# cure-lab/PnPInversion

Hardware: AMD Instinct MI355X
Metric: edited images/sec @ 512x512, 50 DDIM-inv + 50 denoise steps (higher is better)
Workload: dtype f16 (fp32 accumulate; latents / scheduler math fp32); 1 GPU; single 512x512 image per rank, SD-1.x (seeded synthetic weights), directinversion+p2p, faithful schedule: 650 UNet sample-forwards + 1 VAE encode + 5 VAE decodes per image, Refine+Reweight+LocalBlend controller; text K/V projected once per loop (not per forward); ddim_steps=50, schedule=lockstep

## Files before the change

include/pnpi.h:

```cpp
#ifndef PNPI_H
#define PNPI_H
#include <stddef.h>
#include <stdint.h>

#ifdef __cplusplus
extern "C" {
#endif

typedef struct pnpi_ctx pnpi_ctx;

typedef enum {
  PNPI_OK = 0,
  PNPI_EINVAL = -1,
  PNPI_ESHAPE = -2,
  PNPI_EHIP = -3,
  PNPI_ESTATE = -4,
  PNPI_ENOMEM = -5
} pnpi_status;

typedef struct {
  int in_channels, out_channels;
  int n_blocks;
  int block_out_channels[4];
  int block_has_attn[4];
// ... 188 lines not shown
int pnpi_op_adam_step(pnpi_ctx* ctx, float* p, float* m, float* v, const float* g, int n, int k, float lr, float inv_scale);
int pnpi_op_attention_bwd(pnpi_ctx* ctx, const void* q, int ldq, int q_off, const void* k, int ldk, int k_off, const void* v, int ldv,
                          int v_off, const void* d_o, int ldo, int heads, int Nq, int Nk, int Dp, int dh, float scale, int B, void* dq,
                          void* dk, void* dv, void* scratch, size_t scratch_bytes);
size_t pnpi_op_attention_bwd_scratch_bytes(int Nq, int Nk, int dh);

int pnpi_edit_loop_uncond_steps(pnpi_ctx* ctx, const float* x_T, int nimg, const float* context4, const pnpi_ctrl_desc* ctrl_host, int nsteps,
                                const int* timesteps_host, float guidance_scale, int prox, float quantile, const float* uncond_steps,
                                int uncond_first_only, float* latents_out);
int pnpi_edit_loop_uncond_steps_recon(pnpi_ctx* ctx, const float* x_T, int nimg, const float* context4, const pnpi_ctrl_desc* ctrl_host, int nsteps,
                                      const int* timesteps_host, float guidance_scale, int prox, float quantile, const float* uncond_steps,
                                      int uncond_first_only, const pnpi_recon_desc* recon, float* latents_out);
int pnpi_unet_context_grad(pnpi_ctx* ctx, const float* latents, int t, const float* context, const float* d_eps, float* eps_out,
                           float* d_context_out);
int pnpi_null_text_optimize(pnpi_ctx* ctx, const float* ddim_latents, const float* ctx_uncond, const float* ctx_cond, int nsteps,
                            const int* timesteps_host, float guidance_scale, int num_inner_steps, float epsilon, float* uncond_out,
                            int* iters_out_host, float* losses_out_host);
int pnpi_null_latent_calculate(pnpi_ctx* ctx, const float* ddim_latents, const float* context4, int nsteps, const int* timesteps_host,
                               float guidance_scale, int num_inner_steps, float epsilon, float* noise_loss_out, int* iters_out_host,
                               float* losses_out_host);
int pnpi_op_attention(pnpi_ctx* ctx, const void* q, int ldq, int q_off, const void* k, int ldk, int k_off, const void* vt,
                      int ldv, void* o, int ldo, int heads, int Nq, int Nk, int Dp, int dh, float scale,
                      const int* rows_dev , int nrows);
int pnpi_op_cross_edit(pnpi_ctx* ctx, const void* q, int ldq, int q_off, const void* k, int ldk, int k_off, const void* vt,
                       int ldv, void* o, int ldo, int heads, int Nq, int Nk, int Dp, int dh, float scale,
                       const int* pairs_dev, int npairs, const void* mmatT_f16, const float* c1, const float* c2,
                       const float* lb_alpha, float* lb_acc, int lb_slot0, int lb_nslots);
int pnpi_op_local_blend(pnpi_ctx* ctx, const float* lb_acc, int nslots, int map_hw, int lat_hw, int C, float th,
                        float* latents, int nimg);
int pnpi_op_local_blend_sub(pnpi_ctx* ctx, const float* lb_acc, int nslots, int map_hw, int lat_hw, int C, float th, float th_sub,
                            float* latents, int nimg);

#ifdef __cplusplus
}
#endif
#endif
```

pnpinversion_amd/_capi.py:

```python
import ctypes as C
import os

_HERE = os.path.dirname(os.path.abspath(__file__))
LIB_PATH = os.path.join(_HERE, "csrc", "libpnpi.so")

PNPI_OK, PNPI_EINVAL, PNPI_ESHAPE, PNPI_EHIP, PNPI_ESTATE, PNPI_ENOMEM = 0, -1, -2, -3, -4, -5


class ModelConfig(C.Structure):
    _fields_ = [
        ("in_channels", C.c_int), ("out_channels", C.c_int), ("n_blocks", C.c_int),
        ("block_out_channels", C.c_int * 4), ("block_has_attn", C.c_int * 4),
        ("layers_per_block", C.c_int), ("heads", C.c_int), ("cross_dim", C.c_int), ("ctx_len", C.c_int),
        ("sample_size", C.c_int), ("norm_groups", C.c_int), ("n_train_timesteps", C.c_int),
        ("vae_in_channels", C.c_int), ("vae_latent_channels", C.c_int), ("vae_n_blocks", C.c_int),
        ("vae_block_out_channels", C.c_int * 4), ("vae_layers_per_block", C.c_int), ("vae_norm_groups", C.c_int),
        ("clip_layers", C.c_int), ("clip_heads", C.c_int), ("clip_intermediate", C.c_int), ("clip_vocab", C.c_int),
    ]


class NamedTensor(C.Structure):
    _fields_ = [("name", C.c_char_p), ("data", C.c_void_p), ("dtype", C.c_int), ("ndim", C.c_int), ("shape", C.c_int64 * 4)]


# ... 83 lines not shown
    "pnpi_op_gemm_geglu": (_i, [_vp, _vp, _i, _vp, _i, _i, _i, _i, _vp, _vp, _i]),
    "pnpi_op_groupnorm": (_i, [_vp, _vp, _vp, _i, _i, _i, _i, _i, _f, _vp, _vp, _i, _vp]),
    "pnpi_op_layernorm": (_i, [_vp, _vp, _i, _i, _f, _vp, _vp, _vp]),
    "pnpi_op_geglu": (_i, [_vp, _vp, _i, _i, _vp]),
    "pnpi_op_softmax_rows": (_i, [_vp, _vp, _i, _i, _i]),
    "pnpi_op_layernorm_bwd": (_i, [_vp, _vp, _vp, _i, _i, _f, _vp, _vp]),
    "pnpi_op_groupnorm_bwd": (_i, [_vp, _vp, _vp, _i, _i, _i, _i, _i, _f, _vp, _vp, _i, _vp, _vp]),
    "pnpi_op_geglu_bwd": (_i, [_vp, _vp, _vp, _i, _i, _vp]),
    "pnpi_op_softmax_bwd_rows": (_i, [_vp, _vp, _vp, _i, _i, _i, _f, _vp]),
    "pnpi_op_accumulate": (_i, [_vp, _vp, _vp, C.c_size_t]),
    "pnpi_op_sumpool2x2": (_i, [_vp, _vp, _i, _i, _i, _i, _vp]),
    "pnpi_op_zero_stuff2": (_i, [_vp, _vp, _i, _i, _i, _i, _vp]),
    "pnpi_op_repack_dgrad": (_i, [_vp, _vp, _i, _i, _i, _vp]),
    "pnpi_op_null_text_loss": (_i, [_vp, _vp, _vp, _vp, _vp, _i, _f, _f, _f, _f, _vp, _vp]),
    "pnpi_op_adam_step": (_i, [_vp, _vp, _vp, _vp, _vp, _i, _i, _f, _f]),
    "pnpi_op_attention_bwd": (_i, [_vp, _vp, _i, _i, _vp, _i, _i, _vp, _i, _i, _vp, _i, _i, _i, _i, _i, _i, _f, _i, _vp, _vp, _vp, _vp, C.c_size_t]),
    "pnpi_op_attention_bwd_scratch_bytes": (C.c_size_t, [_i, _i, _i]),
    "pnpi_edit_loop_uncond_steps": (_i, [_vp, _vp, _i, _vp, _vp, _i, C.POINTER(C.c_int), _f, _i, _f, _vp, _i, _vp]),
    "pnpi_edit_loop_uncond_steps_recon": (_i, [_vp, _vp, _i, _vp, _vp, _i, C.POINTER(C.c_int), _f, _i, _f, _vp, _i, C.POINTER(ReconDesc), _vp]),
    "pnpi_unet_context_grad": (_i, [_vp, _vp, _i, _vp, _vp, _vp, _vp]),
    "pnpi_null_text_optimize": (_i, [_vp, _vp, _vp, _vp, _i, C.POINTER(C.c_int), _f, _i, _f, _vp, C.POINTER(C.c_int), C.POINTER(C.c_float)]),
    "pnpi_null_latent_calculate": (_i, [_vp, _vp, _vp, _i, C.POINTER(C.c_int), _f, _i, _f, _vp, C.POINTER(C.c_int), C.POINTER(C.c_float)]),
    "pnpi_op_attention": (_i, [_vp, _vp, _i, _i, _vp, _i, _i, _vp, _i, _vp, _i, _i, _i, _i, _i, _i, _f, _vp, _i]),
    "pnpi_op_cross_edit": (_i, [_vp, _vp, _i, _i, _vp, _i, _i, _vp, _i, _vp, _i, _i, _i, _i, _i, _i, _f, _vp, _i, _vp, _vp,
                                _vp, _vp, _vp, _i, _i]),
    "pnpi_op_local_blend": (_i, [_vp, _vp, _i, _i, _i, _i, _f, _vp, _i]),
    "pnpi_op_local_blend_sub": (_i, [_vp, _vp, _i, _i, _i, _i, _f, _f, _vp, _i]),
    "pnpi_ef_step_scalars": (_i, [_fp, _i, _f, _i, _i, _f, _fp]),
    "pnpi_ef_sample_xts": (_i, [_vp, _vp, _i, _vp, _sz, _i, _ip, _vp]),
    "pnpi_ef_noise_map": (_i, [_vp, _vp, _i, _f, _vp, _vp, _vp, _i, _sz, _i, _i, _f]),
    "pnpi_ef_reverse_step": (_i, [_vp, _vp, _vp, _vp, _i, _i, _sz, _fp, _i, _i, _f, _vp]),
    "pnpi_ef_invert": (_i, [_vp, _vp, _i, _vp, _vp, _vp, _f, _fp, _i, _ip, _vp, _vp]),
    "pnpi_ef_edit": (_i, [_vp, _vp, _vp, _i, _i, _vp, _fp, C.POINTER(CtrlDesc), _fp, _i, _i, _ip, _vp]),
}

_lib = None


class PnpiError(RuntimeError):
    def __init__(self, status, message):
        super().__init__("libpnpi status %d: %s" % (status, message))
        self.status = status


def load_library(path=None):
    global _lib
# ... 28 lines not shown
```

pnpinversion_amd/csrc/api.hip:

```cpp
#include <math.h>
#include <stdio.h>
#include <stdlib.h>
#include <string.h>

#include <algorithm>
#include <functional>
#include <memory>
#include <string>

#include "model.h"

static int g_text_kv = 1;
static int g_temb_cache = 1;

static int fail(pnpi_ctx* c, int status, const char* what) {
  c->err = what;
  return status;
}
static int fail_launch(pnpi_ctx* c, int code, const char* what) {
  char buf[640];
  if (code > 0) {
    snprintf(buf, sizeof(buf), "HIP error %d (%s) in %s", code, hipGetErrorString((hipError_t)code), what);
    c->err = buf;
    return PNPI_EHIP;
// ... 1055 lines not shown
                       int ups, int Ho, int Wo, const void* w, const float* bias, const void* res, int N, void* out, int force_cfg,
                       int force_split, float* stats_out, int* tile_rows_out) {
  if (!c || !stats_out || !tile_rows_out) return PNPI_EINVAL;
  GemmP p; gemm_defaults(p);
  p.x1 = (const half_t*)x1; p.x2 = (const half_t*)x2; p.C1 = C1; p.C2 = C2; p.ldx1 = C1; p.ldx2 = C2;
  p.B = B; p.H = H; p.W = W; p.Ho = Ho; p.Wo = Wo; p.ksize = ksize; p.stride = stride; p.pad = pad; p.ups = ups;
  p.K = ksize * ksize * (C1 + C2); p.w = (const half_t*)w; p.ldw = p.K; p.M = B * Ho * Wo; p.N = N;
  p.bias = bias; p.res = (const half_t*)res; p.ldres = N; p.out = (half_t*)out; p.ldo = N; p.stats = stats_out;
  CK(launch_igemm(p, c->splitk_ws, c->splitk_bytes, c->st, force_cfg, force_split, nullptr, tile_rows_out));
  return 0;
}
int pnpi_tile_table_lookup(int M, int N, int K, int ksize, int* cfg, int* split, int* entry_m) {
  return igemm_table_lookup(M, N, K, ksize, cfg, split, entry_m);
}
int pnpi_set_tuning(const char* key, int value) {
  if (!key) return PNPI_EINVAL;
  if (!strcmp(key, "text_kv")) { g_text_kv = value; return 0; }
  if (!strcmp(key, "temb_cache")) { g_temb_cache = value; return 0; }
  if (!strcmp(key, "gn_inline_rows")) { norm_set_tuning_gn_inline_rows(value); return 0; }
  if (!strcmp(key, "attn_vt_perm")) { g_vt_perm = value; return 0; }
  if (!strcmp(key, "attn_aug")) { g_attn_aug = value; return 0; }
  if (!strcmp(key, "attn_pipe")) return attn_set_tuning_pipe(value) == 0 ? 0 : PNPI_EINVAL;
  if (!strcmp(key, "gn_slab")) { g_gn_slab = value; return 0; }
  if (!strcmp(key, "op_attention_aug")) { g_op_attention_aug = value; return 0; }
  if (!strcmp(key, "op_attention_vt_perm")) { g_op_attention_vt_perm = value; return 0; }
  if (!strcmp(key, "attn_bwd_flash")) { g_attn_bwd_flash = value; return 0; }
  return igemm_set_tuning(key, value) == 0 ? 0 : PNPI_EINVAL;
}
int pnpi_op_gemm(pnpi_ctx* c, const void* a, int lda, const void* w, int ldw, int M, int N, int K, float alpha, const float* bias,
                 const void* res, void* out, int ldo, int vt_col0, void* outT, int vt_ld, int vt_f32, int rpb, int force_cfg,
                 int force_split) {
  GemmP p; gemm_defaults(p);
  p.x1 = (const half_t*)a; p.C1 = K; p.ldx1 = lda; p.B = 1; p.H = 1; p.W = M; p.Ho = 1; p.Wo = M; p.ksize = 1;
  p.w = (const half_t*)w; p.ldw = ldw; p.M = M; p.N = N; p.K = K; p.alpha = alpha; p.bias = bias; p.res = (const half_t*)res;
  p.ldres = N; p.out = (half_t*)out; p.ldo = ldo;
  if (outT) { p.outT = outT; p.vt_col0 = vt_col0; p.vt_ld = vt_ld; p.vt_f32 = vt_f32; p.rows_per_batch = rpb; }
  CK(launch_igemm(p, c->splitk_ws, c->splitk_bytes, c->st, force_cfg, force_split));
  return 0;
}
int pnpi_op_gemm_geglu(pnpi_ctx* c, const void* a, int lda, const void* w, int ldw, int M, int N, int K, const float* bias, void* out,
                       int ldo) {
  GemmP p; gemm_defaults(p);
  p.x1 = (const half_t*)a; p.C1 = K; p.ldx1 = lda; p.B = 1; p.H = 1; p.W = M; p.Ho = 1; p.Wo = M; p.ksize = 1;
  p.w = (const half_t*)w; p.ldw = ldw; p.M = M; p.N = N; p.K = K; p.bias = bias; p.out = (half_t*)out; p.ldo = ldo; p.geglu = 1;
  CK(launch_igemm(p, c->splitk_ws, c->splitk_bytes, c->st));
  return 0;
// ... 256 lines not shown
int pnpi_op_repack_dgrad(pnpi_ctx* c, const void* w, int N, int taps, int Cin, void* wd) {
  CK(launch_repack_dgrad((const half_t*)w, N, N, taps, Cin, (half_t*)wd, c->st));
  return 0;
}
int pnpi_op_null_text_loss(pnpi_ctx* c, const float* eps_u, const float* eps_c, const float* x, const float* target, int n, float w, float c_x,
                           float c_e, float grad_scale, void* d_eps_u, float* loss) {
  CK(launch_null_text_loss(eps_u, eps_c, x, target, n, w, c_x, c_e, grad_scale, (float*)d_eps_u, loss, c->st));
  return 0;
}
int pnpi_op_adam_step(pnpi_ctx* c, float* p, float* m, float* v, const float* g, int n, int k, float lr, float inv_scale) {
  CK(launch_adam_step(p, m, v, g, n, k, lr, inv_scale, c->st));
  return 0;
}
int pnpi_op_attention(pnpi_ctx* c, const void* q, int ldq, int q_off, const void* k, int ldk, int k_off, const void* vt, int ldv,
                      void* o, int ldo, int heads, int Nq, int Nk, int Dp, int dh, float scale, const int* rows_dev, int nrows) {
  AttnP a; a.q = (const half_t*)q; a.ldq = ldq; a.q_off = q_off; a.k = (const half_t*)k; a.ldk = ldk; a.k_off = k_off;
  a.vt = (const half_t*)vt; a.ldv = ldv; a.o = (half_t*)o; a.ldo = ldo; a.heads = heads; a.Nq = Nq; a.Nk = Nk; a.Dp = Dp; a.dh = dh;
  a.scale = scale; a.rows = rows_dev; a.nrows = nrows;
  a.vt_perm = (g_op_attention_vt_perm && attn_flash_uses_dma64(Dp, Nk, 0)) ? 1 : 0;
  a.aug = g_op_attention_aug;
  CK(launch_attn_flash(a, c->st));
  return 0;
}
int pnpi_op_cross_edit(pnpi_ctx* c, const void* q, int ldq, int q_off, const void* k, int ldk, int k_off, const void* vt, int ldv,
                       void* o, int ldo, int heads, int Nq, int Nk, int Dp, int dh, float scale, const int* pairs_dev, int npairs,
                       const void* mmatT, const float* c1, const float* c2, const float* lb_alpha, float* lb_acc, int lb_slot0,
                       int lb_nslots) {
  CrossEditP e; e.q = (const half_t*)q; e.ldq = ldq; e.q_off = q_off; e.k = (const half_t*)k; e.ldk = ldk; e.k_off = k_off;
  e.vt = (const half_t*)vt; e.ldv = ldv; e.o = (half_t*)o; e.ldo = ldo; e.heads = heads; e.Nq = Nq; e.Nk = Nk; e.Dp = Dp; e.dh = dh;
  e.scale = scale; e.pairs = pairs_dev; e.npairs = npairs; e.mmatT = (const half_t*)mmatT; e.c1 = c1; e.c2 = c2;
  e.lb_alpha = lb_alpha; e.lb_acc = lb_acc; e.lb_slot0 = lb_slot0; e.lb_nslots = lb_nslots; e.write_src = 1;
  CK(launch_attn_cross_edit(e, c->st));
  return 0;
}
int pnpi_op_local_blend(pnpi_ctx* c, const float* lb_acc, int nslots, int map_hw, int lat_hw, int C, float th, float* latents, int nimg) {
  CK(launch_local_blend(lb_acc, nslots, map_hw, lat_hw, C, th, latents, nimg, c->st));
  return 0;
}
int pnpi_op_local_blend_sub(pnpi_ctx* c, const float* lb_acc, int nslots, int map_hw, int lat_hw, int C, float th, float th_sub,
                            float* latents, int nimg) {
  CK(launch_local_blend(lb_acc, nslots, map_hw, lat_hw, C, th, latents, nimg, c->st, 4, th_sub));
  return 0;
}

}
```

pnpinversion_amd/csrc/api_ctrl.inc:

```
static void for_each_transformer(pnpi_ctx* c, const std::function<void(const TransformerW&, int)>& fn) {
  UNetW& u = c->unet;
  int idx = 0;
  for (auto& blk : u.down_attn) for (auto& t : blk) fn(t, idx++);
  fn(u.mid_attn, idx++);
  for (auto& blk : u.up_attn) for (auto& t : blk) fn(t, idx++);
}
static size_t text_kv_bytes(pnpi_ctx* c, int rows) {
  const int T = c->cfg.ctx_len, ldv = round_up_i(T, 8);
  size_t total = 0;
  for_each_transformer(c, [&](const TransformerW& t, int) {
    const size_t hd = (size_t)t.heads * t.Dp;
    total += align_up((size_t)rows * T * hd * sizeof(half_t), 256) + align_up((size_t)rows * hd * ldv * sizeof(half_t), 256);
  });
  return total + 4096;
}
static int text_kv_precompute(pnpi_ctx* c, const float* context, int rows) {
  const pnpi_model_config& g = c->cfg;
  TextKV& kv = c->tkv;
  kv.rows = 0; kv.use = false;
  if (rows <= 0 || rows > c->max_rows) return fail(c, PNPI_EINVAL, "text K/V precompute: rows out of range (max_unet_rows)");
  if (text_kv_bytes(c, rows) > kv.cap) return fail(c, PNPI_ENOMEM, "text K/V cache arena too small");
  const int T = g.ctx_len, X = g.cross_dim, ldv = round_up_i(T, 8);
  c->persist.reset(); c->temp.reset();
  half_t* ctx16 = palloc(c, (size_t)rows * T * X);
// ... 50 lines not shown
      if (step_list) step_on.assign(cds[i].masa_step_on_host, cds[i].masa_step_on_host + cds[i].masa_n_steps);
      if (cd.masa_any && (cd.masa_start_step != cds[i].masa_start_step || cd.masa_start_layer != cds[i].masa_start_layer ||
                          cd.masa_layer_mask != cds[i].masa_layer_mask || cd.masa_step_list != step_list || cd.masa_step_on != step_on))
        return fail(c, PNPI_EINVAL, "all MasaCtrl controllers of one batch must share their step / layer windows (or lists)");
      cd.masa_any = true; cd.masa_start_step = cds[i].masa_start_step; cd.masa_start_layer = cds[i].masa_start_layer;
      cd.masa_layer_mask = cds[i].masa_layer_mask; cd.masa_step_list = step_list; cd.masa_step_on = step_on;
      for (int half = 0; half < 2; ++half) {
        const int src = i * 4 + 2 * half, tgt = src + 1;
        masa[tgt * 4 + 2] = src; masa[tgt * 4 + 3] = src;
      }
    }
    if (cd.masa_any) {
      cd.rows_masa = (int*)c->ctrl_arena.alloc(masa.size() * sizeof(int));
      CKP(upload(c, cd.rows_masa, masa.data(), masa.size() * sizeof(int)));
    }
  }
  cd.any_edit = !edit_img.empty();
  cd.npairs = (int)edit_img.size();
  std::vector<bool> is_pair_row(rows, false);
  for (int i : edit_img) {
    int src = i * rpi + src_off, tgt = i * rpi + tgt_off;
    rep[tgt * 4 + 1] = src; rep[tgt * 4 + 2] = src;
    pairs.push_back(src); pairs.push_back(tgt);
    is_pair_row[tgt] = true;
    cd.pair_img.push_back(i);
  }
  for (int r = 0; r < rows; ++r) if (!is_pair_row[r]) { plain.push_back(r); plain.push_back(r); plain.push_back(r); plain.push_back(r); }
  cd.n_plain = (int)plain.size() / 4;
  cd.rows_id = (int*)c->ctrl_arena.alloc(id.size() * sizeof(int));
  cd.rows_rep = (int*)c->ctrl_arena.alloc(rep.size() * sizeof(int));
  CKP(upload(c, cd.rows_id, id.data(), id.size() * sizeof(int)));
  CKP(upload(c, cd.rows_rep, rep.data(), rep.size() * sizeof(int)));
  if (!plain.empty()) {
    cd.rows_plain = (int*)c->ctrl_arena.alloc(plain.size() * sizeof(int));
    CKP(upload(c, cd.rows_plain, plain.data(), plain.size() * sizeof(int)));
  }
  if (!cd.any_edit) return 0;
  cd.pairs = (int*)c->ctrl_arena.alloc(pairs.size() * sizeof(int));
  CKP(upload(c, cd.pairs, pairs.data(), pairs.size() * sizeof(int)));
  const pnpi_ctrl_desc& d0 = cds[edit_img[0]];
  cd.n_alpha_rows = d0.n_alpha_rows;
  cd.self_lo = d0.self_replace_lo; cd.self_hi = d0.self_replace_hi; cd.self_max_tokens = d0.self_replace_max_tokens;
  const int P = cd.npairs;
  std::vector<half_t> mm((size_t)P * 96 * 96, (half_t)0.f);
  int planes = 2;
  for (int pi = 0; pi < P; ++pi)
// ... 64 lines not shown
```

pnpinversion_amd/csrc/api_graph.inc:

```
static void prof_open(pnpi_ctx* c, ProfRec& r) {
  (void)hipEventCreate(&r.a); (void)hipEventCreate(&r.b);
  (void)hipEventRecord(r.a, c->st);
}
static void prof_close(pnpi_ctx* c, ProfRec& r, int cls, double flops, double bytes, int M = 0, int N = 0, int K = 0, int ks = 0) {
  (void)hipEventRecord(r.b, c->st);
  r.cls = cls; r.flops = flops; r.bytes = bytes; r.M = M; r.N = N; r.K = K; r.ksize = ks;
  c->prof.push_back(r);
}
static int g_gn_slab = 0;
static int flush_pending(pnpi_ctx* c) {
  if (!c->pend_on) return 0;
  c->pend_on = false;
  return launch_splitk_reduce(c->pend, c->st);
}
#define PROF(cls, flops, bytes, expr) PROFD(cls, flops, bytes, 0, 0, 0, expr)
#define PROFD(cls, flops, bytes, d0, d1, d2, expr)            \
  do {                                                        \
    if (c->pend_on) { int _f = flush_pending(c); if (_f) return fail_launch(c, _f, "deferred split-K combine"); } \
    if (c->prof_on && !c->dry) {                              \
      ProfRec _pr; prof_open(c, _pr);                         \
      int _r = (expr);                                        \
      prof_close(c, _pr, (cls), (flops), (bytes), (d0), (d1), (d2)); \
      if (_r) return fail_launch(c, _r, #expr);               \
    } else {                                                  \
// ... 15 lines not shown
  const NormW* nw = nullptr;
  int G = 0, HW = 0, silu = 0;
  float eps = 0.f;
  const half_t *q = nullptr, *k = nullptr, *v = nullptr;
  const float* lse = nullptr;
  int ldq = 0, q_off = 0, ldk = 0, k_off = 0, ldv = 0, v_off = 0, heads = 0, Nq = 0, Nk = 0, Dp = 0, dh = 0;
  float scale = 0.f;
};
struct Tape {
  std::vector<TapeOp> ops;
  bool rec = false;
  const half_t* no_grad_input = nullptr;
  const half_t* ctx16 = nullptr;
  Bump garena;
  std::unordered_map<const void*, half_t*> grads;
  std::unordered_map<const void*, half_t*> wd;
  float* d_ctx = nullptr;
  void* attn_scratch = nullptr; size_t attn_scratch_bytes = 0;
};
static int g_attn_aug = 1;
static int g_vt_perm = 1;
static int g_attn_bwd_flash = 1;
static int g_op_attention_aug = 0;
static int g_op_attention_vt_perm = 0;
static inline bool taping(pnpi_ctx* c) { return c->tape && c->tape->rec && !c->dry; }
static inline bool keep_acts(pnpi_ctx* c) { return c->tape && c->tape->rec; }

struct Stats { const float* p = nullptr; int rows = 0; };
struct StatsReq { float* buf = nullptr; int rows = 0; bool transient = false; };

static half_t* talloc(pnpi_ctx* c, size_t n) { return (half_t*)c->temp.alloc(n * sizeof(half_t)); }
static half_t* palloc(pnpi_ctx* c, size_t n) { return (half_t*)c->persist.alloc(n * sizeof(half_t)); }

static int op_gn(pnpi_ctx* c, const half_t* x1, const half_t* x2, int C1, int C2, int B, int HW, const NormW& nw, int G, float eps,
                 int silu, half_t* out, Stats s1 = Stats(), Stats s2 = Stats()) {
  if (c->dry) return 0;
  if (taping(c)) {
    TapeOp o; o.kind = TK_GN; o.x1 = x1; o.x2 = x2; o.C1 = C1; o.C2 = C2; o.B = B; o.HW = HW; o.nw = &nw; o.G = G; o.eps = eps; o.silu = silu; o.out = out;
    c->tape->ops.push_back(o);
  }
  if (c->pend_on) {
    const GemmP& q = c->pend;
    if (q.out == x1 && q.N == C1 && q.ldo == C1 && q.M == B * HW && !taping(c) && groupnorm_slab_ok(C1, C2, HW, G) && (C2 == 0 || x2)) {
      c->pend_on = false;
      GnSlab sl; sl.slab = q.slab; sl.splitk = q.splitk; sl.stride = (size_t)q.M * q.N; sl.bias = q.bias; sl.res = q.res; sl.ldres = q.ldres;
      sl.sum_out = c->pend_keep ? q.out : nullptr;
// ... 165 lines not shown
  const int vperm = (g_vt_perm && !c->attn_cb && N % 16 == 0 && attn_flash_uses_dma64(t.Dp, N, 0)) ? 1 : 0;
  {
    VtOut v; v.outT = vt; v.col0 = 2 * hd; v.ld = ldv; v.f32 = 0; v.rpb = N; v.perm16 = vperm;
    CK(op_gemm(c, n1, C, M, C, t.w_qkv, C, 3 * hd, t.b_qkv_aug, nullptr, 0, qk, 2 * hd, 1.f, &v, 2.0 * M * 3.0 * C * C));
  }
  half_t* ao = talloc(c, (size_t)M * C);
  {
    AttnP a; a.q = qk; a.ldq = 2 * hd; a.q_off = 0; a.k = qk; a.ldk = 2 * hd; a.k_off = hd; a.vt = vt; a.ldv = ldv; a.vt_perm = vperm;
    a.aug = (t.b_qkv_aug && g_attn_aug) ? 1 : 0;
    a.o = ao; a.ldo = C; a.heads = t.heads; a.Nq = N; a.Nk = N; a.Dp = t.Dp; a.dh = t.dh; a.scale = scale;
    const bool rep = edit && cur_step >= cd.self_lo && cur_step < cd.self_hi && N <= cd.self_max_tokens;
    const bool masa_step = cd.masa_step_list ? (cur_step >= 0 && cur_step < (int)cd.masa_step_on.size() && cd.masa_step_on[cur_step]) : cur_step >= cd.masa_start_step;
    const bool masa_layer = cd.masa_layer_mask ? ((cd.masa_layer_mask >> block_index) & 1u) != 0 && block_index < 31 : block_index >= cd.masa_start_layer;
    const bool masa = use_ctrl && cd.masa_any && masa_step && masa_layer;
    a.rows = rep ? cd.rows_rep : (masa ? cd.rows_masa : cd.rows_id); a.nrows = B;
    c->ctr.executed_attn_flops += 4.0 * B * t.heads * (double)N * N * t.Dp;
    if (c->attn_cb && !c->dry) {
      CKP(attn_materialized(c, qk, 2 * hd, 0, qk, 2 * hd, hd, vt, ldv, ao, C, t.heads, N, N, t.Dp, t.dh, scale, B, 0, t.place, 2 * block_index));
    } else if (!c->dry) PROFD(PNPI_KC_ATTN_FLASH, 4.0 * B * t.heads * (double)N * N * t.dh, 0.0, N, N, t.Dp, launch_attn_flash(a, c->st));
  }
  half_t* hs1 = talloc(c, (size_t)M * C);
  CK(op_gemm(c, ao, C, M, C, t.o1.w, C, C, t.o1.b, hs, C, hs1, C));

  half_t* n2 = talloc(c, (size_t)M * C);
  if (!c->dry) PROF(PNPI_KC_LAYERNORM, 0.0, 2.0 * M * (double)C * 2.0, launch_layernorm(hs1, M, C, 1e-5f, t.ln2.g, t.ln2.b, n2, c->st));
  half_t* q2 = talloc(c, (size_t)M * hd);
  CK(op_gemm(c, n2, C, M, C, t.w_q2, C, hd, nullptr, nullptr, 0, q2, hd, 1.f, nullptr, 2.0 * M * (double)C * C));
  const int ldv2 = round_up_i(T, 8);
  half_t *k2, *vt2;
  if (c->tkv.use) {
    k2 = c->tkv.k[block_index]; vt2 = c->tkv.vt[block_index];
  } else {
    k2 = talloc(c, (size_t)B * T * hd);
    vt2 = talloc(c, (size_t)B * hd * ldv2);
    if (c->attn_cb && !c->dry && ldv2 != T) CKH(hipMemsetAsync(vt2, 0, (size_t)B * hd * ldv2 * sizeof(half_t), c->st));
    VtOut v; v.outT = vt2; v.col0 = hd; v.ld = ldv2; v.f32 = 0; v.rpb = T;
    CK(op_gemm(c, ctx16, X, B * T, X, t.w_kv2, X, 2 * hd, nullptr, nullptr, 0, k2, hd, 1.f, &v, 2.0 * B * T * 2.0 * C * X));
  }
  half_t* ao2 = talloc(c, (size_t)M * C);
  {
    AttnP a; a.q = q2; a.ldq = hd; a.q_off = 0; a.k = k2; a.ldk = hd; a.k_off = 0; a.vt = vt2; a.ldv = ldv2;
    a.o = ao2; a.ldo = C; a.heads = t.heads; a.Nq = N; a.Nk = T; a.Dp = t.Dp; a.dh = t.dh; a.scale = scale;
    a.rows = edit ? cd.rows_plain : cd.rows_id; a.nrows = edit ? cd.n_plain : B;
    c->ctr.executed_attn_flops += 4.0 * B * t.heads * (double)N * 96 * t.Dp;
    if (c->attn_cb && !c->dry) {
      CKP(attn_materialized(c, q2, hd, 0, k2, hd, 0, vt2, ldv2, ao2, C, t.heads, N, T, t.Dp, t.dh, scale, B, 1, t.place, 2 * block_index + 1));
    } else if (!c->dry) PROFD(PNPI_KC_ATTN_FLASH, 4.0 * a.nrows * t.heads * (double)N * T * t.dh, 0.0, N, T, t.Dp, launch_attn_flash(a, c->st));
    if (edit && !c->dry && !c->attn_cb) {
      CrossEditP e; e.q = q2; e.ldq = hd; e.q_off = 0; e.k = k2; e.ldk = hd; e.k_off = 0; e.vt = vt2; e.ldv = ldv2;
      e.o = ao2; e.ldo = C; e.heads = t.heads; e.Nq = N; e.Nk = T; e.Dp = t.Dp; e.dh = t.dh; e.scale = scale;
      e.pairs = cd.pairs; e.npairs = cd.npairs; e.mmatT = cd.mmatT;
      int srow = cur_step < cd.n_alpha_rows ? cur_step : cd.n_alpha_rows - 1;
      e.c1 = cd.coef + ((size_t)srow * 2 + 0) * cd.npairs * 96;
      e.c2 = cd.coef + ((size_t)srow * 2 + 1) * cd.npairs * 96;
      const bool lb = cd.lb_any && t.lb_slot0 >= 0 && N == c->unet.lb_tokens;
      e.lb_alpha = lb ? cd.lb_alpha : nullptr;
      e.lb_acc = lb ? cd.lb_acc : nullptr;
      e.lb_slot0 = t.lb_slot0; e.lb_nslots = c->unet.lb_nslots; e.lb_planes = cd.lb_planes; e.write_src = 0;
      PROF(PNPI_KC_ATTN_EDIT, 4.0 * 2 * cd.npairs * t.heads * (double)N * T * t.dh, 0.0, launch_attn_cross_edit(e, c->st));
    }
  }
  half_t* hs2 = talloc(c, (size_t)M * C);
  CK(op_gemm(c, ao2, C, M, C, t.o2.w, C, C, t.o2.b, hs1, C, hs2, C));

  half_t* n3 = talloc(c, (size_t)M * C);
  if (!c->dry) PROF(PNPI_KC_LAYERNORM, 0.0, 2.0 * M * (double)C * 2.0, launch_layernorm(hs2, M, C, 1e-5f, t.ln3.g, t.ln3.b, n3, c->st));
  half_t* f2 = talloc(c, (size_t)M * 4 * C);
  if (C % 64 == 0) {
    CK(op_gemm(c, n3, C, M, C, t.ff1.w, C, 8 * C, t.ff1.b, nullptr, 0, f2, 4 * C, 1.f, nullptr, -1.0, 1));
// ... 364 lines not shown
```

pnpinversion_amd/csrc/attn.hip:

```cpp
#include <stdlib.h>

#include "ops.h"

static constexpr int KV_TILE = 64;
static constexpr int SV_LD = KV_TILE + 4;

template <int DP, bool PF>
__global__ void __launch_bounds__(256) attn_flash_kernel(AttnP p) {
  constexpr int KS = DP / 16;
  constexpr int OT = DP / 32;
  constexpr int SK_LD = DP + 8;
  __shared__ __attribute__((aligned(16))) half_t sK[KV_TILE * SK_LD];
  __shared__ __attribute__((aligned(16))) half_t sV[DP * SV_LD];

  const int tid = threadIdx.x, lane = tid & 63, wave = tid >> 6;
  const int h = lane >> 5, ql = lane & 31;
  const int nqt = (p.Nq + 127) >> 7, T = nqt * p.heads * p.nrows, per = (T + 7) >> 3;
  const int tix = (int)(blockIdx.x & 7) * per + (int)(blockIdx.x >> 3);
  if (tix >= T) return;
  const int qt = tix % nqt, head = (tix / nqt) % p.heads;
  const int* rw = p.rows + (tix / (nqt * p.heads)) * 4;
  const int orow = rw[0], qrow = rw[1], krow = rw[2], vrow = rw[3];
  const int qtok = qt * 128 + wave * 32 + ql;
  const bool qok = qtok < p.Nq;
// ... 537 lines not shown
      if (p.vt_perm) attn_flash_dma64_kernel<true, 3><<<grid, 256, 0, st>>>(p);
      else attn_flash_dma64_kernel<false, 3><<<grid, 256, 0, st>>>(p);
    } else {
      if (p.vt_perm) attn_flash_dma64_kernel<true><<<grid, 256, 0, st>>>(p);
      else attn_flash_dma64_kernel<false><<<grid, 256, 0, st>>>(p);
    }
    return (int)hipGetLastError();
  }
  if (p.vt_perm) return -6;
  const bool pf = p.Nk > 2 * KV_TILE;
#define LAUNCH_FLASH(D) (pf ? attn_flash_kernel<D, true><<<grid, 256, 0, st>>>(p) : attn_flash_kernel<D, false><<<grid, 256, 0, st>>>(p))
  switch (p.Dp) {
    case 32: LAUNCH_FLASH(32); break;
    case 64: LAUNCH_FLASH(64); break;
    case 96: LAUNCH_FLASH(96); break;
    case 128: LAUNCH_FLASH(128); break;
    case 160: LAUNCH_FLASH(160); break;
    default: return -5;
  }
#undef LAUNCH_FLASH
  return (int)hipGetLastError();
}

static constexpr int CE_KEYS = 96;
static constexpr int CE_LD = CE_KEYS + 4;

template <int DP>
__global__ void __launch_bounds__(256) attn_cross_edit_kernel(CrossEditP p) {
  constexpr int KS = DP / 16, OT = DP / 32, SK_LD = DP + 8;
  extern __shared__ __attribute__((aligned(16))) char smem_raw[];
  half_t* sK = reinterpret_cast<half_t*>(smem_raw);
  half_t* sV = sK + 2 * CE_KEYS * SK_LD;
  half_t* sM = sV + 2 * DP * CE_LD;
  float* sC = reinterpret_cast<float*>(sM + CE_KEYS * CE_LD);

  const int tid = threadIdx.x, lane = tid & 63, wave = tid >> 6;
  const int h = lane >> 5, ql = lane & 31;
  const int head = blockIdx.y, pair = blockIdx.z;
  const int rows2[2] = {p.pairs[pair * 2 + 0], p.pairs[pair * 2 + 1]};
  const int qtok = blockIdx.x * 128 + wave * 32 + ql;
  const bool qok = qtok < p.Nq;

  half8 qf2[2][KS];
#pragma unroll
  for (int which = 0; which < 2; ++which) {
    const half_t* qp = p.q + ((size_t)rows2[which] * p.Nq + (qok ? qtok : 0)) * p.ldq + p.q_off + head * DP + h * 8;
// ... 507 lines not shown
```

pnpinversion_amd/csrc/model.h:

```cpp
#pragma once
#include <atomic>
#include <string>
#include <unordered_map>
#include <vector>

#include "../../include/pnpi.h"
#include "ops.h"

static inline size_t align_up(size_t x, size_t a) { return (x + a - 1) / a * a; }
static inline int round_up_i(int x, int a) { return (x + a - 1) / a * a; }

struct Bump {
  char* base = nullptr;
  size_t cap = 0, off = 0, peak = 0;
  bool overflow = false;
  void* alloc(size_t bytes) {
    off = align_up(off, 256);
    size_t at = off;
    off += bytes;
    if (off > peak) peak = off;
    if (base && off > cap) { overflow = true; return base; }
    return base ? (void*)(base + at) : (void*)(uintptr_t)(0x1000 + at);
  }
  size_t mark() const { return off; }
// ... 99 lines not shown
struct CtrlDev {
  bool any_edit = false;
  int nimg = 0, n_alpha_rows = 0;
  int npairs = 0;
  int lb_any = 0;
  std::vector<int> lb_start;
  std::vector<float> lb_th;
  std::vector<float> lb_th_sub;
  int lb_planes = 2;
  std::vector<int> lb_enabled;
  std::vector<int> pair_img;
  int self_lo = 0, self_hi = 0, self_max_tokens = 0;
  int* rows_id = nullptr;
  int* rows_rep = nullptr;
  int* rows_plain = nullptr;
  int* rows_masa = nullptr;
  bool masa_any = false;
  int masa_start_step = 0, masa_start_layer = 0;
  unsigned masa_layer_mask = 0;
  std::vector<unsigned char> masa_step_on;
  bool masa_step_list = false;
  int n_plain = 0;
  int* pairs = nullptr;
  half_t* mmatT = nullptr;
  float* coef = nullptr;
  float* lb_alpha = nullptr;
  float* lb_acc = nullptr;
};

struct TextKV {
  std::vector<half_t*> k, vt;
  char* base = nullptr; size_t cap = 0;
  int rows = 0;
  bool use = false;
};

struct ProfRec { int cls; double flops, bytes; hipEvent_t a, b; int M, N, K, ksize; int cfg = -1, split = 0; int geom[7] = {0, 0, 0, 0, 0, 0, 0}; };

struct Tape;

struct pnpi_ctx {
  pnpi_model_config cfg;
  int device;
  hipStream_t st;
  std::string err;
  int max_rows, max_vae;
// ... 40 lines not shown
```

pnpinversion_amd/csrc/ops.h:

```cpp
#pragma once
#include "common.h"

struct GemmP {
  const half_t* x1; const half_t* x2;
  int C1, C2, ldx1, ldx2;
  int B, H, W, Ho, Wo;
  int ksize, stride, pad, ups;
  const half_t* w; int ldw;
  int M, N, K;
  const float* bias;
  const half_t* res; int ldres;
  float alpha;
  half_t* out; int ldo;
  void* outT; int vt_col0, vt_ld, vt_f32, rows_per_batch;
  int vt_perm16;
  float* slab; int splitk, kchunks_per_split;
  float* stats;
  int geglu;
  int epi_lds;
  int bias_init;
  int res_late;
  int k_order;
  int gx, gy, gz, tile_order;
  int nbatch;
// ... 57 lines not shown
  int aug = 0;
  float* lse = nullptr;
};
int launch_attn_flash(const AttnP& p, hipStream_t st);
int attn_set_tuning_pipe(int v);
bool attn_flash_uses_dma64(int Dp, int Nk, int causal);

struct BwdMat { const half_t* p; long hs; int ld; int w; };
struct AttnBwdP {
  BwdMat b1, b2;
  BwdMat l1, l2;
  int nb, nl, heads;
  float scale;
  float* lse;
  float* dsum;
  half_t* out; long out_hs; int out_ld, out_w;
  const half_t* o = nullptr; long o_hs = 0; int o_ld = 0;
  int nsplit = 1;
  float* part = nullptr;
};
int launch_attn_bwd_reduce(const AttnBwdP& p, hipStream_t st);
int launch_attn_bwd_flash(const AttnBwdP& p, int mode , int Dp, hipStream_t st);

struct CrossEditP {
  const half_t* q; int ldq, q_off;
  const half_t* k; int ldk, k_off;
  const half_t* vt; int ldv;
  half_t* o; int ldo;
  int heads, Nq, Nk, Dp, dh;
  float scale;
  const int* pairs;
  int npairs;
  const half_t* mmatT;
  const float* c1; const float* c2;
  const float* lb_alpha;
  float* lb_acc;
  int lb_planes = 2;
  int lb_slot0, lb_nslots;
  int write_src;
};
int launch_attn_cross_edit(const CrossEditP& p, hipStream_t st);

int launch_ddim_move(const float* x, const float* eps, float a_from, float a_to, size_t n, float* out, hipStream_t st);
int launch_ddim_prev_recon(const float* x, const float* eps, float a_from, float a_to, const float* ref, float lr, const float* mask, size_t n,
                           float* out, float* x0_out, hipStream_t st);
int launch_cfg_ddim_prev(const float* eps, const float* x, int nimg, int rows_per_img, size_t row_elems, float gscale,
// ... 37 lines not shown
```

Measured before the change: 1.017 images/s.

## Fuse LayerNorm, Q projection and cross-attention into one kernel

```diff
diff --git a/include/pnpi.h b/include/pnpi.h
--- a/include/pnpi.h
+++ b/include/pnpi.h
@@ -234,6 +234,9 @@
 int pnpi_op_attention(pnpi_ctx* ctx, const void* q, int ldq, int q_off, const void* k, int ldk, int k_off, const void* vt,
                       int ldv, void* o, int ldo, int heads, int Nq, int Nk, int Dp, int dh, float scale,
                       const int* rows_dev , int nrows);
+int pnpi_op_xattn_fused(pnpi_ctx* ctx, const void* x_f16, int C, const float* ln_gamma, const float* ln_beta, float eps, const void* wq_f16,
+                        const void* k, int ldk, int k_off, const void* vt, int ldv, void* o, int ldo, int heads, int Nq, int Nk, int Dp,
+                        int dh, float scale, const int* rows_dev , int nrows, int heads_per_wg);
 int pnpi_op_cross_edit(pnpi_ctx* ctx, const void* q, int ldq, int q_off, const void* k, int ldk, int k_off, const void* vt,
                        int ldv, void* o, int ldo, int heads, int Nq, int Nk, int Dp, int dh, float scale,
                        const int* pairs_dev, int npairs, const void* mmatT_f16, const float* c1, const float* c2,
diff --git a/pnpinversion_amd/_capi.py b/pnpinversion_amd/_capi.py
--- a/pnpinversion_amd/_capi.py
+++ b/pnpinversion_amd/_capi.py
@@ -129,6 +129,7 @@
     "pnpi_null_text_optimize": (_i, [_vp, _vp, _vp, _vp, _i, C.POINTER(C.c_int), _f, _i, _f, _vp, C.POINTER(C.c_int), C.POINTER(C.c_float)]),
     "pnpi_null_latent_calculate": (_i, [_vp, _vp, _vp, _i, C.POINTER(C.c_int), _f, _i, _f, _vp, C.POINTER(C.c_int), C.POINTER(C.c_float)]),
     "pnpi_op_attention": (_i, [_vp, _vp, _i, _i, _vp, _i, _i, _vp, _i, _vp, _i, _i, _i, _i, _i, _i, _f, _vp, _i]),
+    "pnpi_op_xattn_fused": (_i, [_vp, _vp, _i, _vp, _vp, _f, _vp, _vp, _i, _i, _vp, _i, _vp, _i, _i, _i, _i, _i, _i, _f, _vp, _i, _i]),
     "pnpi_op_cross_edit": (_i, [_vp, _vp, _i, _i, _vp, _i, _i, _vp, _i, _vp, _i, _i, _i, _i, _i, _i, _f, _vp, _i, _vp, _vp,
                                 _vp, _vp, _vp, _i, _i]),
     "pnpi_op_local_blend": (_i, [_vp, _vp, _i, _i, _i, _i, _f, _vp, _i]),
diff --git a/pnpinversion_amd/csrc/api.hip b/pnpinversion_amd/csrc/api.hip
--- a/pnpinversion_amd/csrc/api.hip
+++ b/pnpinversion_amd/csrc/api.hip
@@ -1101,6 +1101,7 @@
   if (!strcmp(key, "attn_aug")) { g_attn_aug = value; return 0; }
   if (!strcmp(key, "attn_pipe")) return attn_set_tuning_pipe(value) == 0 ? 0 : PNPI_EINVAL;
   if (!strcmp(key, "gn_slab")) { g_gn_slab = value; return 0; }
+  if (!strcmp(key, "xattn_fuse")) { if (value < 0 || value > 2) return PNPI_EINVAL; g_xattn_fuse = value; return 0; }
   if (!strcmp(key, "op_attention_aug")) { g_op_attention_aug = value; return 0; }
   if (!strcmp(key, "op_attention_vt_perm")) { g_op_attention_vt_perm = value; return 0; }
   if (!strcmp(key, "attn_bwd_flash")) { g_attn_bwd_flash = value; return 0; }
@@ -1403,6 +1404,15 @@
   CK(launch_attn_flash(a, c->st));
   return 0;
 }
+int pnpi_op_xattn_fused(pnpi_ctx* c, const void* x, int C, const float* ln_gamma, const float* ln_beta, float eps, const void* wq, const void* k,
+                        int ldk, int k_off, const void* vt, int ldv, void* o, int ldo, int heads, int Nq, int Nk, int Dp, int dh, float scale,
+                        const int* rows_dev, int nrows, int heads_per_wg) {
+  XAttnP f; f.x = (const half_t*)x; f.C = C; f.ln_g = ln_gamma; f.ln_b = ln_beta; f.eps = eps; f.wq = (const half_t*)wq;
+  f.k = (const half_t*)k; f.ldk = ldk; f.k_off = k_off; f.vt = (const half_t*)vt; f.ldv = ldv; f.o = (half_t*)o; f.ldo = ldo;
+  f.heads = heads; f.Nq = Nq; f.Nk = Nk; f.Dp = Dp; f.dh = dh; f.scale = scale; f.rows = rows_dev; f.nrows = nrows; f.hpw = heads_per_wg;
+  CK(launch_attn_xfused(f, c->st));
+  return 0;
+}
 int pnpi_op_cross_edit(pnpi_ctx* c, const void* q, int ldq, int q_off, const void* k, int ldk, int k_off, const void* vt, int ldv,
                        void* o, int ldo, int heads, int Nq, int Nk, int Dp, int dh, float scale, const int* pairs_dev, int npairs,
                        const void* mmatT, const float* c1, const float* c2, const float* lb_alpha, float* lb_acc, int lb_slot0,
diff --git a/pnpinversion_amd/csrc/api_ctrl.inc b/pnpinversion_amd/csrc/api_ctrl.inc
--- a/pnpinversion_amd/csrc/api_ctrl.inc
+++ b/pnpinversion_amd/csrc/api_ctrl.inc
@@ -96,6 +96,8 @@
     int src = i * rpi + src_off, tgt = i * rpi + tgt_off;
     rep[tgt * 4 + 1] = src; rep[tgt * 4 + 2] = src;
     pairs.push_back(src); pairs.push_back(tgt);
+    if (cd.pair_row_hi < 0) { cd.pair_row_lo = std::min(src, tgt); cd.pair_row_hi = std::max(src, tgt); }
+    cd.pair_row_lo = std::min(cd.pair_row_lo, std::min(src, tgt)); cd.pair_row_hi = std::max(cd.pair_row_hi, std::max(src, tgt));
     is_pair_row[tgt] = true;
     cd.pair_img.push_back(i);
   }
diff --git a/pnpinversion_amd/csrc/api_graph.inc b/pnpinversion_amd/csrc/api_graph.inc
--- a/pnpinversion_amd/csrc/api_graph.inc
+++ b/pnpinversion_amd/csrc/api_graph.inc
@@ -61,6 +61,11 @@
 static int g_vt_perm = 1;
 static int g_attn_bwd_flash = 1;
 static int g_op_attention_aug = 0;
+static int g_xattn_fuse = 1;
+static bool xattn_fuse_pick(int C, int rows) {
+  (void)rows;
+  return C == 320 || C == 640;
+}
 static int g_op_attention_vt_perm = 0;
 static inline bool taping(pnpi_ctx* c) { return c->tape && c->tape->rec && !c->dry; }
 static inline bool keep_acts(pnpi_ctx* c) { return c->tape && c->tape->rec; }
@@ -272,10 +277,19 @@
   half_t* hs1 = talloc(c, (size_t)M * C);
   CK(op_gemm(c, ao, C, M, C, t.o1.w, C, C, t.o1.b, hs, C, hs1, C));
 
+  const bool xfuse = g_xattn_fuse && !c->attn_cb && !keep_acts(c) && attn_xfused_ok(C, t.heads, t.Dp, T) &&
+                     (g_xattn_fuse == 2 || xattn_fuse_pick(C, B));
+  const int r0 = (xfuse && edit) ? cd.pair_row_lo : 0;
+  const int nr = xfuse ? (edit ? cd.pair_row_hi - cd.pair_row_lo + 1 : 0) : B;
   half_t* n2 = talloc(c, (size_t)M * C);
-  if (!c->dry) PROF(PNPI_KC_LAYERNORM, 0.0, 2.0 * M * (double)C * 2.0, launch_layernorm(hs1, M, C, 1e-5f, t.ln2.g, t.ln2.b, n2, c->st));
   half_t* q2 = talloc(c, (size_t)M * hd);
-  CK(op_gemm(c, n2, C, M, C, t.w_q2, C, hd, nullptr, nullptr, 0, q2, hd, 1.f, nullptr, 2.0 * M * (double)C * C));
+  if (nr > 0) {
+    const int Mr = nr * N;
+    half_t* n2r = n2 + (size_t)r0 * N * C;
+    if (!c->dry) PROF(PNPI_KC_LAYERNORM, 0.0, 2.0 * Mr * (double)C * 2.0, launch_layernorm(hs1 + (size_t)r0 * N * C, Mr, C, 1e-5f, t.ln2.g, t.ln2.b, n2r, c->st));
+    CK(op_gemm(c, n2r, C, Mr, C, t.w_q2, C, hd, nullptr, nullptr, 0, q2 + (size_t)r0 * N * hd, hd, 1.f, nullptr, 2.0 * Mr * (double)C * C));
+  }
+  if (nr < B) c->ctr.executed_gemm_flops += 2.0 * (double)(B - nr) * N * hd * C;
   const int ldv2 = round_up_i(T, 8);
   half_t *k2, *vt2;
   if (c->tkv.use) {
@@ -295,6 +309,11 @@
     c->ctr.executed_attn_flops += 4.0 * B * t.heads * (double)N * 96 * t.Dp;
     if (c->attn_cb && !c->dry) {
       CKP(attn_materialized(c, q2, hd, 0, k2, hd, 0, vt2, ldv2, ao2, C, t.heads, N, T, t.Dp, t.dh, scale, B, 1, t.place, 2 * block_index + 1));
+    } else if (xfuse && !c->dry) {
+      XAttnP f; f.x = hs1; f.C = C; f.ln_g = t.ln2.g; f.ln_b = t.ln2.b; f.eps = 1e-5f; f.wq = t.w_q2;
+      f.k = k2; f.ldk = hd; f.k_off = 0; f.vt = vt2; f.ldv = ldv2; f.o = ao2; f.ldo = C; f.heads = t.heads; f.Nq = N; f.Nk = T; f.Dp = t.Dp;
+      f.dh = t.dh; f.scale = scale; f.rows = a.rows; f.nrows = a.nrows;
+      PROFD(PNPI_KC_ATTN_FLASH, a.nrows * (double)N * (4.0 * t.heads * T * t.dh + 2.0 * C * C), 0.0, N, T, t.Dp, launch_attn_xfused(f, c->st));
     } else if (!c->dry) PROFD(PNPI_KC_ATTN_FLASH, 4.0 * a.nrows * t.heads * (double)N * T * t.dh, 0.0, N, T, t.Dp, launch_attn_flash(a, c->st));
     if (edit && !c->dry && !c->attn_cb) {
       CrossEditP e; e.q = q2; e.ldq = hd; e.q_off = 0; e.k = k2; e.ldk = hd; e.k_off = 0; e.vt = vt2; e.ldv = ldv2;
diff --git a/pnpinversion_amd/csrc/attn.hip b/pnpinversion_amd/csrc/attn.hip
--- a/pnpinversion_amd/csrc/attn.hip
+++ b/pnpinversion_amd/csrc/attn.hip
@@ -583,6 +583,274 @@
   return (int)hipGetLastError();
 }
 
+template <int DP> struct XfGeom { static constexpr int WR = DP > 128 ? 1 : 2, KC = DP > 128 ? 32 : 64; };
+
+template <int DP>
+__global__ void __launch_bounds__(256) attn_xfused_kernel(XAttnP p) {
+  constexpr int WR = XfGeom<DP>::WR, WH = 4 / WR, RT = 32 * WR, KC = XfGeom<DP>::KC, OT = DP / 32;
+  constexpr int SW_LD = KC + 8, SK_LD = DP + 8, SVT_LD = 32 + 4;
+  static_assert(DP % 32 == 0 && (WH * DP * (KC / 8)) % 256 == 0, "a weight chunk is a whole number of 16-byte vectors per thread");
+  static_assert(DP * SW_LD >= 32 * SK_LD && DP * SW_LD >= DP * SVT_LD, "the K / V^T tiles fit the weight-chunk buffer");
+  extern __shared__ __attribute__((aligned(16))) char smem_raw[];
+  const int SN_LD = p.C + 8;
+  half_t* sN = reinterpret_cast<half_t*>(smem_raw);
+  half_t* sB = sN + RT * SN_LD;
+
+  const int tid = threadIdx.x, lane = tid & 63, wave = tid >> 6;
+  const int h = lane >> 5, ql = lane & 31;
+  const int nqt = (p.Nq + RT - 1) / RT;
+  const int qt = blockIdx.x % nqt;
+  const int* rw = p.rows + (blockIdx.x / nqt) * 4;
+  const int orow = rw[0], qrow = rw[1], krow = rw[2], vrow = rw[3];
+
+  {
+    const int C8 = p.C >> 3;
+    bool ok[4];
+#pragma unroll
+    for (int i = 0; i < 4; ++i) ok[i] = lane + 64 * i < C8;
+    for (int r0 = wave * (RT / 4); r0 < (wave + 1) * (RT / 4); r0 += 2) {
+      half8 v[2][4];
+#pragma unroll
+      for (int r = 0; r < 2; ++r) {
+        const half_t* src = p.x + ((size_t)qrow * p.Nq + min(qt * RT + r0 + r, p.Nq - 1)) * p.C;
+#pragma unroll
+        for (int i = 0; i < 4; ++i) v[r][i] = ldg_half8(src + min(lane + 64 * i, C8 - 1) * 8);
+      }
+      float s[2], q[2];
+#pragma unroll
+      for (int r = 0; r < 2; ++r) {
+        s[r] = 0.f;
+#pragma unroll
+        for (int i = 0; i < 4; ++i)
+          if (ok[i]) {
+#pragma unroll
+            for (int j = 0; j < 8; ++j) s[r] += (float)v[r][i][j];
+          }
+      }
+#pragma unroll
+      for (int r = 0; r < 2; ++r) s[r] = wave_sum(s[r]);
+#pragma unroll
+      for (int r = 0; r < 2; ++r) {
+        const float mean = s[r] / (float)p.C;
+        s[r] = mean;
+        q[r] = 0.f;
+#pragma unroll
+        for (int i = 0; i < 4; ++i)
+          if (ok[i]) {
+#pragma unroll
+            for (int j = 0; j < 8; ++j) { float d = (float)v[r][i][j] - mean; q[r] += d * d; }
+          }
+      }
+#pragma unroll
+      for (int r = 0; r < 2; ++r) q[r] = wave_sum(q[r]);
+#pragma unroll
+      for (int i = 0; i < 4; ++i) {
+        if (!ok[i]) continue;
+        const int c0 = (lane + 64 * i) * 8;
+        float ga[8], be[8];
+#pragma unroll
+        for (int j = 0; j < 8; ++j) { ga[j] = p.ln_g[c0 + j]; be[j] = p.ln_b[c0 + j]; }
+#pragma unroll
+        for (int r = 0; r < 2; ++r) {
+          const float mean = s[r], rstd = rsqrtf(q[r] / (float)p.C + p.eps);
+          half8 o;
+#pragma unroll
+          for (int j = 0; j < 8; ++j) o[j] = (half_t)(((float)v[r][i][j] - mean) * rstd * ga[j] + be[j]);
+          *reinterpret_cast<half8*>(sN + (r0 + r) * SN_LD + c0) = o;
+        }
+      }
+    }
+  }
+
+  const int wr = wave % WR, wh = wave / WR;
+  const int qtok = qt * RT + wr * 32 + ql;
+  const bool qok = qtok < p.Nq;
+  const float c = p.scale * 1.44269504088896340736f;
+  const half_t* nrow = sN + (wr * 32 + ql) * SN_LD + h * 8;
+
+  for (int hg = 0; hg < p.hpw; hg += WH) {
+    const int head0 = blockIdx.y * p.hpw + hg, head = head0 + wh;
+    floatx16 acc[OT];
+#pragma unroll
+    for (int ot = 0; ot < OT; ++ot)
+#pragma unroll
+      for (int r = 0; r < 16; ++r) acc[ot][r] = 0.f;
+    constexpr int NWV = WH * DP * (KC / 8) / 256;
+    half8 wv[NWV];
+    const half_t* wbase = p.wq + (size_t)head0 * DP * p.C;
+    auto wload = [&](int k0) {
+#pragma unroll
+      for (int i = 0; i < NWV; ++i) {
+        const int idx = tid + i * 256, row = idx / (KC / 8), v = idx - row * (KC / 8);
+        wv[i] = ldg_half8(wbase + (size_t)row * p.C + k0 + v * 8);
+      }
+    };
+    wload(0);
+    for (int k0 = 0; k0 < p.C; k0 += KC) {
+      __syncthreads();
+#pragma unroll
+      for (int i = 0; i < NWV; ++i) {
+        const int idx = tid + i * 256, row = idx / (KC / 8), v = idx - row * (KC / 8);
+        *reinterpret_cast<half8*>(sB + row * SW_LD + v * 8) = wv[i];
+      }
+      __syncthreads();
+      if (k0 + KC < p.C) wload(k0 + KC);
+#pragma unroll
+      for (int ks = 0; ks < KC / 16; ++ks) {
+        const half8 bf = *reinterpret_cast<const half8*>(nrow + k0 + ks * 16);
+#pragma unroll
+        for (int ot = 0; ot < OT; ++ot) {
+          const half8 af = *reinterpret_cast<const half8*>(sB + (wh * DP + ot * 32 + ql) * SW_LD + ks * 16 + h * 8);
+          acc[ot] = mfma32(af, bf, acc[ot]);
+        }
+      }
+    }
+    half8 qf[OT][2];
+#pragma unroll
+    for (int ot = 0; ot < OT; ++ot)
+#pragma unroll
+      for (int r = 0; r < 16; ++r) qf[ot][r >> 3][r & 7] = (half_t)acc[ot][r];
+
+    floatx16 s[3];
+#pragma unroll
+    for (int st = 0; st < 3; ++st) {
+      __syncthreads();
+      for (int idx = tid; idx < WH * 32 * (DP / 8); idx += 256) {
+        const int hh = idx / (32 * (DP / 8)), i = idx - hh * (32 * (DP / 8)), r = i / (DP / 8), v = i - r * (DP / 8);
+        const int key = st * 32 + r;
+        const half8 val = key < p.Nk ? ldg_half8(p.k + ((size_t)krow * p.Nk + key) * p.ldk + p.k_off + (head0 + hh) * DP + v * 8) : zero_half8();
+        *reinterpret_cast<half8*>(sB + (hh * 32 + r) * SK_LD + v * 8) = val;
+      }
+      __syncthreads();
+#pragma unroll
+      for (int r = 0; r < 16; ++r) s[st][r] = 0.f;
+#pragma unroll
+      for (int ot = 0; ot < OT; ++ot)
+#pragma unroll
+        for (int t = 0; t < 2; ++t) {
+          const half_t* kb = sB + (wh * 32 + ql) * SK_LD + ot * 32 + t * 16 + 4 * h;
+          const half4 lo = *reinterpret_cast<const half4*>(kb);
+          const half4 hi = *reinterpret_cast<const half4*>(kb + 8);
+          const half8 kf = {lo[0], lo[1], lo[2], lo[3], hi[0], hi[1], hi[2], hi[3]};
+          s[st] = mfma32(kf, qf[ot][t], s[st]);
+        }
+    }
+    float mx = -INFINITY;
+#pragma unroll
+    for (int st = 0; st < 3; ++st)
+#pragma unroll
+      for (int r = 0; r < 16; ++r) {
+        if (st * 32 + acc_row(r, lane) >= p.Nk) s[st][r] = -INFINITY;
+        mx = fmaxf(mx, s[st][r]);
+      }
+    mx = fmaxf(mx, __shfl_xor(mx, 32, 64));
+    const float mc = mx * c;
+    float psum = 0.f;
+    half8 pf[3][2];
+#pragma unroll
+    for (int st = 0; st < 3; ++st)
+#pragma unroll
+      for (int r = 0; r < 16; ++r) {
+        const float pv = __builtin_amdgcn_exp2f(__builtin_fmaf(s[st][r], c, -mc));
+        psum += pv;
+        pf[st][r >> 3][r & 7] = (half_t)pv;
+      }
+    const float inv = 1.f / (psum + __shfl_xor(psum, 32, 64));
+
+    floatx16 O[OT];
+#pragma unroll
+    for (int ot = 0; ot < OT; ++ot)
+#pragma unroll
+      for (int r = 0; r < 16; ++r) O[ot][r] = 0.f;
+#pragma unroll
+    for (int st = 0; st < 3; ++st) {
+      __syncthreads();
+      for (int idx = tid; idx < WH * DP * 4; idx += 256) {
+        const int row = idx >> 2, v = idx & 3, hh = row / DP, d = row - hh * DP;
+        const int tok0 = st * 32 + v * 8;
+        const half_t* src = p.vt + (((size_t)vrow * p.heads + head0 + hh) * DP + d) * (size_t)p.ldv + tok0;
+        half8 val;
+        if (tok0 + 8 <= p.Nk) {
+          val = ldg_half8(src);
+        } else {
+#pragma unroll
+          for (int j = 0; j < 8; ++j) val[j] = (tok0 + j < p.Nk) ? src[j] : (half_t)0.f;
+        }
+        const half4 lo = {val[0], val[1], val[2], val[3]}, hi = {val[4], val[5], val[6], val[7]};
+        half_t* dst = sB + row * SVT_LD + v * 8;
+        *reinterpret_cast<half4*>(dst) = lo;
+        *reinterpret_cast<half4*>(dst + 4) = hi;
+      }
+      __syncthreads();
+#pragma unroll
+      for (int ot = 0; ot < OT; ++ot)
+#pragma unroll
+        for (int t = 0; t < 2; ++t) {
+          const half_t* vb = sB + (wh * DP + ot * 32 + ql) * SVT_LD + t * 16 + 4 * h;
+          const half4 lo = *reinterpret_cast<const half4*>(vb);
+          const half4 hi = *reinterpret_cast<const half4*>(vb + 8);
+          const half8 vf = {lo[0], lo[1], lo[2], lo[3], hi[0], hi[1], hi[2], hi[3]};
+          O[ot] = mfma32(vf, pf[st][t], O[ot]);
+        }
+    }
+    if (qok) {
+      half_t* op = p.o + ((size_t)orow * p.Nq + qtok) * p.ldo + head * p.dh;
+#pragma unroll
+      for (int ot = 0; ot < OT; ++ot)
+#pragma unroll
+        for (int g = 0; g < 4; ++g) {
+          const int d = ot * 32 + 8 * g + 4 * h;
+          if (d + 3 < p.dh) {
+            half4 o4 = {(half_t)(O[ot][4 * g] * inv), (half_t)(O[ot][4 * g + 1] * inv), (half_t)(O[ot][4 * g + 2] * inv),
+                        (half_t)(O[ot][4 * g + 3] * inv)};
+            *reinterpret_cast<half4*>(op + d) = o4;
+          } else {
+#pragma unroll
+            for (int j = 0; j < 4; ++j)
+              if (d + j < p.dh) op[d + j] = (half_t)(O[ot][4 * g + j] * inv);
+          }
+        }
+    }
+  }
+}
+
+template <int DP>
+static int launch_xf(XAttnP p, hipStream_t st) {
+  constexpr int WR = XfGeom<DP>::WR, WH = 4 / WR, RT = 32 * WR, KC = XfGeom<DP>::KC;
+  if (p.C % KC || p.heads % WH) return -3;
+  const int tiles = ((p.Nq + RT - 1) / RT) * p.nrows;
+  if (p.hpw <= 0) {
+    p.hpw = p.heads;
+    while (p.hpw % (2 * WH) == 0 && tiles * (p.heads / p.hpw) < 256) p.hpw /= 2;
+  }
+  if (p.hpw % WH || p.heads % p.hpw) return -3;
+  const size_t lds = ((size_t)RT * (p.C + 8) + (size_t)WH * DP * (KC + 8)) * sizeof(half_t);
+  if (lds > 160 * 1024) return -3;
+  static DeviceOnce attr_once;
+  if (int r = once_per_device(attr_once, [&]() { return (int)hipFuncSetAttribute((const void*)attn_xfused_kernel<DP>, hipFuncAttributeMaxDynamicSharedMemorySize, 160 * 1024); })) return r;
+  attn_xfused_kernel<DP><<<dim3((unsigned)tiles, (unsigned)(p.heads / p.hpw)), 256, lds, st>>>(p);
+  return (int)hipGetLastError();
+}
+
+bool attn_xfused_ok(int C, int heads, int Dp, int Nk) {
+  if (Dp != 64 && Dp != 96 && Dp != 160) return false;
+  const int kc = Dp > 128 ? 32 : 64, wh = Dp > 128 ? 4 : 2, rt = Dp > 128 ? 32 : 64;
+  return C % kc == 0 && C <= 2048 && heads % wh == 0 && Nk > 0 && Nk <= 96 &&
+         ((size_t)rt * (C + 8) + (size_t)wh * Dp * (kc + 8)) * sizeof(half_t) <= 160 * 1024;
+}
+
+int launch_attn_xfused(const XAttnP& p, hipStream_t st) {
+  if (p.nrows <= 0) return 0;
+  if (!attn_xfused_ok(p.C, p.heads, p.Dp, p.Nk)) return -5;
+  if ((p.ldk & 7) || (p.ldv & 7) || (p.k_off & 7) || (p.dh & 3) || (p.ldo & 3) || p.dh > p.Dp || p.heads * p.dh > p.ldo) return -3;
+  switch (p.Dp) {
+    case 64: return launch_xf<64>(p, st);
+    case 96: return launch_xf<96>(p, st);
+    case 160: return launch_xf<160>(p, st);
+    default: return -5;
+  }
+}
+
 static constexpr int CE_KEYS = 96;
 static constexpr int CE_LD = CE_KEYS + 4;
 
diff --git a/pnpinversion_amd/csrc/model.h b/pnpinversion_amd/csrc/model.h
--- a/pnpinversion_amd/csrc/model.h
+++ b/pnpinversion_amd/csrc/model.h
@@ -145,6 +145,7 @@
   bool masa_step_list = false;
   int n_plain = 0;
   int* pairs = nullptr;
+  int pair_row_lo = 0, pair_row_hi = -1;
   half_t* mmatT = nullptr;
   float* coef = nullptr;
   float* lb_alpha = nullptr;
diff --git a/pnpinversion_amd/csrc/ops.h b/pnpinversion_amd/csrc/ops.h
--- a/pnpinversion_amd/csrc/ops.h
+++ b/pnpinversion_amd/csrc/ops.h
@@ -103,6 +103,22 @@
 int launch_attn_bwd_reduce(const AttnBwdP& p, hipStream_t st);
 int launch_attn_bwd_flash(const AttnBwdP& p, int mode , int Dp, hipStream_t st);
 
+struct XAttnP {
+  const half_t* x; int C;
+  const float* ln_g; const float* ln_b; float eps;
+  const half_t* wq;
+  const half_t* k; int ldk, k_off;
+  const half_t* vt; int ldv;
+  half_t* o; int ldo;
+  int heads, Nq, Nk, Dp, dh;
+  float scale;
+  const int* rows;
+  int nrows;
+  int hpw = 0;
+};
+bool attn_xfused_ok(int C, int heads, int Dp, int Nk);
+int launch_attn_xfused(const XAttnP& p, hipStream_t st);
+
 struct CrossEditP {
   const half_t* q; int ldq, q_off;
   const half_t* k; int ldk, k_off;
```

Result: slower. 0.9776 images/s (-3.9%).
